# kemingy/rabitq

Hardware: AMD Instinct MI355X
Metric: queries/sec at recall@10>=0.95, 100Mx128; HBM GB/s on popcount scan (higher is better)
Workload: dtype exact integer dot (fp6 MFMA, v_dot8_u32_u4) + f32

## Files before the change

rabitq_amd/csrc/host_state.h:

```cpp
#pragma once
static thread_local std::string g_err;
static rq_status fail(rq_status s, const std::string &msg) {
    g_err = msg;
    return s;
}
#define HIPC(expr)                                                                                   \
    do {                                                                                             \
        hipError_t _e = (expr);                                                                      \
        if (_e != hipSuccess)                                                                        \
            return fail(_e == hipErrorOutOfMemory ? RQ_ERR_OOM : RQ_ERR_HIP,                         \
                        std::string(#expr) + ": " + hipGetErrorString(_e));                          \
    } while (0)
#define RQC(expr)                        \
    do {                                 \
        rq_status _s = (expr);           \
        if (_s != RQ_OK) return _s;      \
    } while (0)

static rq_status ensure_device() {
    int count = 0;
    hipError_t e = hipGetDeviceCount(&count);
    if (e != hipSuccess || count == 0)
        return fail(RQ_ERR_NO_DEVICE, "no HIP device visible (librabitq_hip has no CPU fallback)");
    return RQ_OK;
// ... 373 lines not shown
    if (cnt[b] == topk) {
        m = dist[(uint64_t)b * topk];
        for (uint32_t e = 1; e < topk; ++e) m = dist[(uint64_t)b * topk + e] > m ? dist[(uint64_t)b * topk + e] : m;
    }
    thr[b] = m;
}
__global__ void pack_topk_keys_at_kernel(const float *__restrict__ dist, const uint32_t *__restrict__ id, const uint32_t *__restrict__ cnt,
                                         uint32_t nq, uint32_t topk, uint32_t id_offset, uint32_t width, uint32_t col0,
                                         unsigned long long *__restrict__ keys) {
    const uint64_t i = (uint64_t)blockIdx.x * blockDim.x + threadIdx.x;
    if (i >= (uint64_t)nq * topk) return;
    const uint32_t b = (uint32_t)(i / topk), e = (uint32_t)(i - (uint64_t)b * topk);
    keys[(uint64_t)b * width + col0 + e] =
        e < cnt[b] ? (((unsigned long long)ord32_biased(dist[i]) << 32) | (uint32_t)(id[i] + id_offset)) : ~0ull;
}
__global__ void unpack_topk_keys_kernel(const unsigned long long *__restrict__ keys, uint32_t nq, uint32_t topk,
                                        float *__restrict__ dist, uint32_t *__restrict__ id, uint32_t *__restrict__ cnt) {
    const uint32_t b = blockIdx.x * blockDim.x + threadIdx.x;
    if (b >= nq) return;
    uint32_t c = 0;
    for (uint32_t e = 0; e < topk; ++e) {
        const unsigned long long key = keys[(uint64_t)b * topk + e];
        if (key == ~0ull) break;
        dist[(uint64_t)b * topk + e] = ord32_unbias((uint32_t)(key >> 32));
        id[(uint64_t)b * topk + e] = (uint32_t)key;
        ++c;
    }
    cnt[b] = c;
}

static std::atomic<int> g_coarse_impl{0};
static std::atomic<int> g_scan_dbg{0};
static bool select_is_wave(uint32_t k, uint32_t nprobe, uint32_t nq) { return nprobe <= 64 && k <= 4096 && nq >= 8; }
static void launch_coarse(const float *cent_t, const float *y, float *dist, uint32_t k, uint32_t dim, uint32_t nq,
                          uint32_t kstride, hipStream_t st) {
    const int impl = g_coarse_impl.load();
    const bool sreg = (impl == 2 || (impl == 0 && nq >= 2048)) && nq > 0;
    if (g_scan_dbg.load() & 16384)
        fprintf(stderr, "[rabitq_hip] plan: coarse=exact kernel=%s nq=%u k=%u\n", sreg ? "sreg" : (nq >= 64 && dim <= 2048 ? "lds8" : "lds4"), nq, k);
    if (sreg)
        coarse_dist_sreg_kernel<8><<<dim3(ceil_div(nq, 8), ceil_div(k, 256)), 256, 0, st>>>(cent_t, y, dist, k, dim, nq, kstride);
    else if (nq >= 64 && dim <= 2048)
        coarse_dist_kernel<8><<<dim3(ceil_div(nq, 8), ceil_div(k, 256)), 256, 8 * dim * sizeof(float), st>>>(cent_t, y, dist, k, dim, nq,
                                                                                                    kstride);
    else
        coarse_dist_kernel<4><<<dim3(ceil_div(nq, 4), ceil_div(k, 256)), 256, 4 * dim * sizeof(float), st>>>(cent_t, y, dist, k, dim, nq,
                                                                                                    kstride);
}

template <typename F>
static void with_row_kpl(uint32_t k, F f) {
    if (k <= 1024) f(std::integral_constant<int, 16>{});
    else if (k <= 4096) f(std::integral_constant<int, 64>{});
    else f(std::integral_constant<int, 128>{});
}
static void launch_select(const float *dist, uint32_t k, uint32_t nprobe, uint32_t *out_cluster, float *out_dist,
                          uint32_t id_offset, uint32_t out_stride, uint32_t nq, hipStream_t st) {
    if (select_is_wave(k, nprobe, nq)) {
        with_row_kpl(k, [&](auto kpl) {
            select_probe_wave_kernel<decltype(kpl)::value><<<ceil_div(nq, 4), 256, 0, st>>>(dist, k, nprobe, out_cluster, out_dist, id_offset, out_stride, nq);
        });
        return;
    }
    select_probe_kernel<<<nq, 256, (size_t)nprobe * 8, st>>>(dist, k, nprobe, out_cluster, out_dist, id_offset, out_stride);
}

static std::atomic<int> g_pair_split{1};
static std::atomic<int> g_coarse_tiled_from{4096};
static bool coarse_prefilter_has(uint32_t W) { return W == 1 || W == 2 || W == 3 || W == 4 || W == 6 || W == 8 || W == 12; }
static bool coarse_prefilter_applies(const rq_index *idx, uint32_t nq, uint32_t nprobe) {
    const int impl = g_coarse_impl.load();
    return (impl == 3 || impl == 4 || (impl == 0 && nq >= 2048)) && coarse_prefilter_has(idx->W) && std::isfinite(idx->cent_norm_max) &&
           idx->cent_bf.p != nullptr && nprobe <= 64 && nq >= 8 && idx->k >= 64 && nprobe >= 1 && idx->k <= 65536;
}
template <int W, int NT>
static size_t coarse_candidates_lds_bytes(uint32_t ntile) { return assign_lds_bytes<W, NT>() + (size_t)4 * NT * 32 * ntile * 4; }
#define RQ_LDS_PER_BLOCK (160u * 1024u)
static bool coarse_fused_applies(const rq_index *idx, uint32_t nprobe, bool have_redo) {
    const uint32_t k = idx->k, ntile = ceil_div(k, 32u);
    if (g_coarse_impl.load() != 0 || (g_scan_dbg.load() & 65536) || !have_redo || k < 4096 || k > 8192 || idx->W > 4 || ntile < nprobe) return false;
    const size_t images = 2 * (32 * ((size_t)idx->dim * 2 + 16) + 128);
    return images + (size_t)4 * 32 * ntile * 4 <= RQ_LDS_PER_BLOCK;
}
static void launch_coarse_prefiltered(const rq_index *idx, const float *y, float *dist, uint32_t nq, uint32_t nprobe, uint32_t *out_cluster,
                                      float *out_dist, uint32_t out_stride, unsigned long long *fallback_rows, uint32_t *redo, hipStream_t st,
                                      uint16_t *y_bf) {
    const uint32_t k = idx->k, dim = idx->dim;
    if (coarse_fused_applies(idx, nprobe, redo != nullptr)) {
        const uint32_t ntile = ceil_div(k, 32u);
        if (g_scan_dbg.load() & 16384) fprintf(stderr, "[rabitq_hip] plan: coarse=prefilter_fused nq=%u k=%u nprobe=%u\n", nq, k, nprobe);
#define RQ_CCK(WW, NT)                                                                                                                   \
    coarse_candidates_kernel<WW, NT><<<ceil_div(nq, 128 * NT), 256, coarse_candidates_lds_bytes<WW, NT>(ntile), st>>>(                   \
        y, idx->cent_bf.p, idx->cent_sqnorm.p, idx->cent_norm_max, nq, k, nprobe, dist, redo)
        if (idx->W == 1 && coarse_candidates_lds_bytes<1, 2>(ntile) <= RQ_LDS_PER_BLOCK) RQ_CCK(1, 2);
        else if (idx->W == 2 && coarse_candidates_lds_bytes<2, 2>(ntile) <= RQ_LDS_PER_BLOCK) RQ_CCK(2, 2);
        else if (idx->W == 1) RQ_CCK(1, 1);
        else if (idx->W == 2) RQ_CCK(2, 1);
        else if (idx->W == 3) RQ_CCK(3, 1);
        else RQ_CCK(4, 1);
#undef RQ_CCK
        refine_candidates_kernel<<<ceil_div(nq, 4), 256, 0, st>>>(dist, y, idx->centroids.p, k, dim, nprobe, out_cluster, out_dist, out_stride, nq, redo,
                                                                  fallback_rows);
        select_probe_kernel<<<nq, 256, (size_t)nprobe * 8, st>>>(dist, k, nprobe, out_cluster, out_dist, 0u, out_stride, redo);
        return;
    }
    if (idx->W > 8) to_bf16_kernel<<<ceil_div((uint64_t)nq * dim / 8, 256), 256, 0, st>>>(y, (uint64_t)nq * dim, y_bf);
#define RQ_CAP(WW, NT)                                                                                                      \
    coarse_approx_kernel<WW, NT><<<ceil_div(nq, 128 * NT), 256, assign_lds_bytes<WW, NT>(), st>>>(y, idx->cent_bf.p, idx->cent_sqnorm.p, nq, \
                                                                                                  k, dist, y_bf)
    switch (idx->W) {
        case 1: RQ_CAP(1, 2); break;
        case 2: RQ_CAP(2, 2); break;
        case 3: RQ_CAP(3, 1); break;
        case 4: RQ_CAP(4, 1); break;
        case 6: RQ_CAP(6, 1); break;
        case 8: RQ_CAP(8, 1); break;
        default: RQ_CAP(12, 1); break;
    }
#undef RQ_CAP
    const dim3 g(ceil_div(nq, 4)), b(256);
    const uint32_t ntile = ceil_div(k, 32u);
    const int impl = g_coarse_impl.load();
    const bool tiled = redo != nullptr && ntile >= nprobe &&
                       (k > 8192 || impl == 4 || (impl != 3 && k >= (uint32_t)g_coarse_tiled_from.load() && idx->W <= 8));
    if (g_scan_dbg.load() & 16384)
        fprintf(stderr, "[rabitq_hip] plan: coarse=%s nq=%u k=%u nprobe=%u\n", tiled ? "prefilter_tiled" : "prefilter_regs", nq, k, nprobe);
    if (tiled) {
#define RQ_TILED(TPL)                                                                                                             \
    select_refine_tiled_kernel<TPL><<<g, b, 4 * 64 * (TPL) * 4, st>>>(dist, y, idx->centroids.p, idx->cent_norm_max, k, dim, nprobe, out_cluster, \
                                                                    out_dist, out_stride, nq, redo, fallback_rows)
        if (ntile <= 128) RQ_TILED(2);
        else if (ntile <= 256) RQ_TILED(4);
        else if (ntile <= 512) RQ_TILED(8);
        else if (ntile <= 1024) RQ_TILED(16);
        else RQ_TILED(32);
#undef RQ_TILED
        select_probe_kernel<<<nq, 256, (size_t)nprobe * 8, st>>>(dist, k, nprobe, out_cluster, out_dist, 0u, out_stride, redo);
    } else {
        with_row_kpl(k, [&](auto kpl) {
            select_refine_wave_kernel<decltype(kpl)::value><<<g, b, 0, st>>>(dist, y, idx->centroids.p, idx->cent_norm_max, k, dim, nprobe, out_cluster, out_dist,
                                                                             out_stride, nq, fallback_rows);
        });
    }
}

#define RQ_MAX_BLOCKS_256 ((1u << 23) - 1)

static void launch_rotate(const float *x, const float *P, float *out, uint64_t n, uint32_t dim, bool mfma,
                          hipStream_t st) {
    const uint64_t rows_per_launch = mfma ? (1ull << 40) : (uint64_t)RQ_MAX_BLOCKS_256 * 4;
    for (uint64_t r0 = 0; r0 < n; r0 += rows_per_launch) {
        const uint64_t m = std::min(rows_per_launch, n - r0);
        const float *xs = x + r0 * dim;
        float *os = out + r0 * dim;
        if (mfma) {
            const uint32_t ncol = dim / ROT_BN;
            const uint64_t nrow_tiles = ceil_div(m, ROT_BM);
            const uint32_t groups = (uint32_t)std::min<uint64_t>(nrow_tiles, std::max<uint32_t>(1, 512 / ncol));
            rotate_mfma_kernel<<<dim3(groups * ncol), dim3(256), 0, st>>>(xs, P, os, m, dim, groups);
        } else {
            rotate_valu_kernel<<<dim3(ceil_div(m, 4), dim / 64), dim3(64, 4), 0, st>>>(xs, P, os, m, dim);
        }
    }
}

static const uint4 *get_tile_table(const rq_index *cidx, uint32_t tile, uint32_t *count) {
    rq_index *idx = const_cast<rq_index *>(cidx);
    std::lock_guard<std::mutex> lk(idx->tt_mu);
    auto it = idx->tile_tables.find(tile);
    if (it == idx->tile_tables.end()) {
        std::vector<uint4> h;
        h.reserve(idx->n / tile + idx->k + 1);
        for (uint32_t c = 0; c < idx->k; ++c) {
            const uint32_t b = idx->h_offsets[c], len = idx->h_offsets[c + 1] - b;
            for (uint32_t f = 0; f < len; f += tile) h.push_back(make_uint4(c, f, b, len));
        }
        std::unique_ptr<DevBuf<uint4>> buf(new DevBuf<uint4>());
        if (buf->alloc(h.size()) != RQ_OK) return nullptr;
        if (!h.empty() && hipMemcpy(buf->p, h.data(), h.size() * sizeof(uint4), hipMemcpyHostToDevice) != hipSuccess) return nullptr;
        buf->count = h.size();
        it = idx->tile_tables.emplace(tile, std::move(buf)).first;
    }
    *count = (uint32_t)it->second->count;
// ... 121 lines not shown
            default: break;
        }
    });
}
static void launch_scan_mfma(const ScanPtrs &p, const ScanArgs &args, uint32_t W, hipStream_t st, bool additive = false) {
    if (p.filtered) {
        if (p.arena) launch_scan_mfma_a<true, true>(p, args, W, st);
        else launch_scan_mfma_a<false, true>(p, args, W, st);
    } else if (p.arena) launch_scan_mfma_a<true>(p, args, W, st);
    else if (additive) launch_scan_mfma_add(p, args, W, st);
    else launch_scan_mfma_a<false>(p, args, W, st);
}

static bool scan_is_fused(uint32_t W) {
    switch (W) {
        case 1: case 2: case 3: case 4: case 6: case 8: case 12: case 16: return true;
        default: return false;
    }
}
static uint32_t scan_tile(uint32_t W) {
    switch (W) {
        case 1: case 2: case 3: case 4: case 6: case 8: return 512;
        default: return 256;
    }
}

template <int W, int NT>
static hipError_t set_scan_mfma_attr() {
    hipError_t e = hipFuncSetAttribute(reinterpret_cast<const void *>(scan_mfma_kernel<W, NT, false>),
                                       hipFuncAttributeMaxDynamicSharedMemorySize, (int)scan_mfma_ring_bytes(W));
    if (e != hipSuccess) return e;
    if constexpr (W <= 2) {
        e = hipFuncSetAttribute(reinterpret_cast<const void *>(scan_mfma_kernel<W, (W == 2 ? RQ_ADD_NT2 : NT), false, true>),
                                hipFuncAttributeMaxDynamicSharedMemorySize, (int)scan_mfma_ring_bytes(W));
        if (e != hipSuccess) return e;
    }
    e = hipFuncSetAttribute(reinterpret_cast<const void *>(scan_mfma_kernel<W, NT, true>),
                            hipFuncAttributeMaxDynamicSharedMemorySize, (int)scan_mfma_ring_bytes(W));
    if (e != hipSuccess) return e;
    e = hipFuncSetAttribute(reinterpret_cast<const void *>(scan_mfma_kernel<W, NT, false, false, true>),
                            hipFuncAttributeMaxDynamicSharedMemorySize, (int)scan_mfma_ring_bytes(W));
    if (e != hipSuccess) return e;
    return hipFuncSetAttribute(reinterpret_cast<const void *>(scan_mfma_kernel<W, NT, true, false, true>),
                               hipFuncAttributeMaxDynamicSharedMemorySize, (int)scan_mfma_ring_bytes(W));
}
void launch_sb_query_filtered(uint32_t W, int mode, uint32_t nq, size_t dyn, hipStream_t st, const SbArgs &sa);
hipError_t sb_query_filtered_set_attributes(int bytes);
static rq_status ensure_kernel_attributes() {
    static std::once_flag once;
    static hipError_t err = hipSuccess;
    static const char *what = "";
    std::call_once(once, [] {
        auto set = [&](const void *fn, int bytes, const char *name) {
            if (err != hipSuccess) return;
            err = hipFuncSetAttribute(fn, hipFuncAttributeMaxDynamicSharedMemorySize, bytes);
            if (err != hipSuccess) what = name;
        };
        set(reinterpret_cast<const void *>(select_probe_kernel), 140 * 1024, "select_probe_kernel");
        set(reinterpret_cast<const void *>(coarse_dist_kernel<4>), 140 * 1024, "coarse_dist_kernel<4>");
        set(reinterpret_cast<const void *>(coarse_dist_kernel<8>), 140 * 1024, "coarse_dist_kernel<8>");
        set(reinterpret_cast<const void *>(assign_generic_kernel<8>), 140 * 1024, "assign_generic_kernel<8>");
        set(reinterpret_cast<const void *>(merge_smallest_u64_kernel), 16384 * 8, "merge_smallest_u64_kernel");
        set(reinterpret_cast<const void *>(group_rank_kernel), 32768 * 4, "group_rank_kernel");
        set(reinterpret_cast<const void *>(sb_front_kernel), 140 * 1024, "sb_front_kernel");
        set(reinterpret_cast<const void *>(accurate_ring8_kernel<RQ_RING_V, 4>), 156 * 1024, "accurate_ring8_kernel<4>");
        set(reinterpret_cast<const void *>(accurate_ring8_kernel<RQ_RING_V, 8>), 156 * 1024, "accurate_ring8_kernel<8>");
        set(reinterpret_cast<const void *>(accurate_ring8_kernel<RQ_RING_V, 12>), 156 * 1024, "accurate_ring8_kernel<12>");
        set(reinterpret_cast<const void *>(accurate_ring8_kernel<RQ_RING_V, 16>), 156 * 1024, "accurate_ring8_kernel<16>");
        set(reinterpret_cast<const void *>(sort_runs_mid_kernel), RQ_SORT_MID_LDS_WORDS * 8, "sort_runs_mid_kernel");
        set(reinterpret_cast<const void *>(range_sort_block_kernel<1024, RQ_RANGE_TILE>), RQ_RANGE_TILE * 8, "range_sort_block_kernel");
        set(reinterpret_cast<const void *>(range_sort_tile_kernel), RQ_RANGE_TILE * 8, "range_sort_tile_kernel");
        set(reinterpret_cast<const void *>(assign_approx_kernel<6, 1>), (int)assign_lds_bytes<6, 1>(), "assign_approx_kernel<6,1>");
        set(reinterpret_cast<const void *>(assign_approx_kernel<8, 1>), (int)assign_lds_bytes<8, 1>(), "assign_approx_kernel<8,1>");
        set(reinterpret_cast<const void *>(assign_approx_kernel<12, 1>), (int)assign_lds_bytes<12, 1>(), "assign_approx_kernel<12,1>");
        set(reinterpret_cast<const void *>(coarse_approx_kernel<6, 1>), (int)assign_lds_bytes<6, 1>(), "coarse_approx_kernel<6,1>");
        set(reinterpret_cast<const void *>(coarse_approx_kernel<8, 1>), (int)assign_lds_bytes<8, 1>(), "coarse_approx_kernel<8,1>");
        set(reinterpret_cast<const void *>(coarse_approx_kernel<12, 1>), (int)assign_lds_bytes<12, 1>(), "coarse_approx_kernel<12,1>");
        set(reinterpret_cast<const void *>(coarse_candidates_kernel<1, 2>), (int)RQ_LDS_PER_BLOCK, "coarse_candidates_kernel<1,2>");
        set(reinterpret_cast<const void *>(coarse_candidates_kernel<2, 2>), (int)RQ_LDS_PER_BLOCK, "coarse_candidates_kernel<2,2>");
        set(reinterpret_cast<const void *>(coarse_candidates_kernel<1, 1>), (int)RQ_LDS_PER_BLOCK, "coarse_candidates_kernel<1,1>");
        set(reinterpret_cast<const void *>(coarse_candidates_kernel<2, 1>), (int)RQ_LDS_PER_BLOCK, "coarse_candidates_kernel<2,1>");
        set(reinterpret_cast<const void *>(coarse_candidates_kernel<3, 1>), (int)RQ_LDS_PER_BLOCK, "coarse_candidates_kernel<3,1>");
        set(reinterpret_cast<const void *>(coarse_candidates_kernel<4, 1>), (int)RQ_LDS_PER_BLOCK, "coarse_candidates_kernel<4,1>");
        set(reinterpret_cast<const void *>(sb_finish_kernel<true>), 104 * 1024, "sb_finish_kernel");
        set(reinterpret_cast<const void *>(sb_finish_kernel<false>), 104 * 1024, "sb_finish_kernel");
#define RQ_SBQ_ATTR(WW)                                                                                  \
    set(reinterpret_cast<const void *>(sb_query_kernel<WW, 0, false>), 120 * 1024, "sb_query_kernel");   \
    set(reinterpret_cast<const void *>(sb_query_kernel<WW, 1, false>), 120 * 1024, "sb_query_kernel");   \
    set(reinterpret_cast<const void *>(sb_query_kernel<WW, 2, false>), 120 * 1024, "sb_query_kernel")
        RQ_SBQ_ATTR(1);
        RQ_SBQ_ATTR(2);
        RQ_SBQ_ATTR(4);
        RQ_SBQ_ATTR(8);
        RQ_SBQ_ATTR(12);
        RQ_SBQ_ATTR(16);
#undef RQ_SBQ_ATTR
        if (err == hipSuccess && (err = sb_query_filtered_set_attributes(120 * 1024)) != hipSuccess) what = "sb_query_kernel (filtered)";
        auto chk = [&](hipError_t e, const char *name) {
            if (err == hipSuccess && e != hipSuccess) err = e, what = name;
        };
        chk(set_scan_mfma_attr<1, 4>(), "scan_mfma_kernel<1,4>");
        chk(set_scan_mfma_attr<2, RQ_NT_W2>(), "scan_mfma_kernel<2,NT>");
        chk(set_scan_mfma_attr<3, 4>(), "scan_mfma_kernel<3,4>");
        chk(set_scan_mfma_attr<4, 2>(), "scan_mfma_kernel<4,2>");
        chk(set_scan_mfma_attr<6, 2>(), "scan_mfma_kernel<6,2>");
        chk(set_scan_mfma_attr<8, 2>(), "scan_mfma_kernel<8,2>");
        chk(set_scan_mfma_attr<12, RQ_NT_W12>(), "scan_mfma_kernel<12,NT>");
        chk(set_scan_mfma_attr<16, 2>(), "scan_mfma_kernel<16,2>");
    });
    if (err != hipSuccess)
        return fail(RQ_ERR_HIP, std::string("hipFuncSetAttribute(") + what + "): " + hipGetErrorString(err));
    return RQ_OK;
}
```

rabitq_amd/csrc/kernels_coarse.h:

```cpp
#pragma once
#ifndef RQ_COLLECT_UNROLL
#define RQ_COLLECT_UNROLL 8
#endif
#include "common.h"

#pragma clang fp contract(off)

template <int QT>
__global__ __launch_bounds__(256) void coarse_dist_sreg_kernel(const float *__restrict__ cent_t,
                                                               const float *__restrict__ y, float *__restrict__ dist,
                                                               uint32_t k, uint32_t dim, uint32_t nq, uint32_t kstride) {
    const uint32_t q0 = blockIdx.x * QT;
    const uint32_t j = blockIdx.y * 256 + threadIdx.x;
    const bool live = j < k;
    const float *cp = cent_t + (live ? j : 0);
    f32x2 acc[QT][4];
#pragma unroll
    for (int v = 0; v < QT; ++v)
#pragma unroll
        for (int l = 0; l < 4; ++l) acc[v][l] = f32x2{0.0f, 0.0f};
    static_assert(QT % 4 == 0, "queries are fetched four at a time");
    for (uint32_t c = 0; c < dim; c += 16) {
        float ce[16];
#pragma unroll
// ... 614 lines not shown
            for (int i = 0; i < (int)(RQ_COARSE_CAND / 64); ++i) kk[i] = lane + 64 * i < base ? (uint32_t)(wn[lane + 64 * i] >> 32) : 0xFFFFFFFFu;
            const uint32_t h2 = bisect_loose(kmin, hi, nprobe, [&](uint32_t t) { return count_le(kk, t); });
            T2 = coarse_margin_key(yr, dim, cmax, ord32_unbias(h2));
            ok = T2 != 0xFFFFFFFFu && collect(T2);
        }
    }
    if (!ok || base < nprobe) {
        coarse_exact_row(centroids, yr, dim, k, d);
        if (lane == 0) {
            redo_flag[b] = 1u;
            if (fallback_rows) atomicAdd(fallback_rows, 1ull);
        }
        return;
    }
    if (lane == 0) redo_flag[b] = 0u;
    __builtin_amdgcn_fence(__ATOMIC_SEQ_CST, "wavefront");
    coarse_refine_tail(wn, base, centroids, yr, dim, nprobe, b, out_cluster, out_dist, out_stride);
}

template <int W, int NT>
__global__ __launch_bounds__(256, (W <= 4 ? 2 : 1)) void coarse_approx_kernel(const float *__restrict__ y ,
                                                              const uint16_t *__restrict__ cent_bf ,
                                                              const float *__restrict__ cnorm, uint32_t nq, uint32_t k,
                                                              float *__restrict__ dist ,
                                                              const uint16_t *__restrict__ y_bf ) {
    constexpr int DIM = 64 * W, NM = DIM / 16;
    constexpr uint32_t ROWB = CentTile<W>::ROWB, TILEB = CentTile<W>::TILEB;
    extern __shared__ __attribute__((aligned(16))) unsigned char asg_lds[];
    const uint32_t t = threadIdx.x, lane = t & 63, wave = t >> 6, col = lane & 31, kh = lane >> 5;
    const uint32_t v0 = (blockIdx.x * 4 + wave) * (32 * NT);
    asg_bf16x8 afrag[NT][NM];
#pragma unroll
    for (int tl = 0; tl < NT; ++tl) {
        const uint32_t v = v0 + 32 * tl + col;
        const uint64_t vr = v < nq ? v : (nq - 1);
        if constexpr (NM > 32) {
            const uint16_t *xb = y_bf + vr * DIM + 8 * kh;
#pragma unroll
            for (int m = 0; m < NM; ++m) afrag[tl][m] = __builtin_bit_cast(asg_bf16x8, *reinterpret_cast<const uint4 *>(xb + 16 * m));
        } else {
        const float *xp = y + vr * DIM + 8 * kh;
#pragma unroll
        for (int m = 0; m < NM; ++m) {
            const float4 a = *reinterpret_cast<const float4 *>(xp + 16 * m), b = *reinterpret_cast<const float4 *>(xp + 16 * m + 4);
            const uint4 pk = make_uint4(asg_bf16_pair(a.x, a.y), asg_bf16_pair(a.z, a.w), asg_bf16_pair(b.x, b.y), asg_bf16_pair(b.z, b.w));
            afrag[tl][m] = __builtin_bit_cast(asg_bf16x8, pk);
        }
        }
    }
    const uint32_t ntile = (k + 31) / 32;
    CentTile<W> next;
    next.stage(cent_bf, cnorm, k, 0, 0.0f);
    next.land(asg_lds, 0);
    for (uint32_t tile = 0; tile < ntile; ++tile) {
        __syncthreads();
        if (tile + 1 < ntile) next.stage(cent_bf, cnorm, k, tile + 1, 0.0f);
        const unsigned char *img = CentTile<W>::image(asg_lds, tile & 1u);
        const float cn = reinterpret_cast<const float *>(img + TILEB)[col];
        asg_f32x16 acc[NT];
#pragma unroll
        for (int tl = 0; tl < NT; ++tl) acc[tl] = asg_f32x16{0, 0, 0, 0, 0, 0, 0, 0, 0, 0, 0, 0, 0, 0, 0, 0};
#pragma unroll
        for (int m = 0; m < NM; ++m) {
            const asg_bf16x8 cf = *reinterpret_cast<const asg_bf16x8 *>(img + col * ROWB + (16 * m + 8 * kh) * 2);
#pragma unroll
            for (int tl = 0; tl < NT; ++tl) acc[tl] = __builtin_amdgcn_mfma_f32_32x32x16_bf16(afrag[tl][m], cf, acc[tl], 0, 0, 0);
        }
        const uint32_t j = 32 * tile + col;
        if (j < k) {
#pragma unroll
            for (int tl = 0; tl < NT; ++tl)
#pragma unroll
                for (int r = 0; r < 16; ++r) {
                    const uint32_t v = v0 + 32 * tl + (uint32_t)((r & 3) + 8 * (r >> 2)) + 4 * kh;
                    if (v < nq) dist[(uint64_t)v * k + j] = fmaf(-2.0f, acc[tl][r], cn);
                }
        }
        if (tile + 1 < ntile) next.land(asg_lds, (tile + 1) & 1u);
    }
}

#define RQ_COARSE_PAD_NORM 3.0e38f
#define RQ_FUSED_WINDOW 4u
template <int W, int NT>
__global__ __launch_bounds__(256) void coarse_candidates_kernel(const float *__restrict__ y ,
                                                                const uint16_t *__restrict__ cent_bf ,
                                                                const float *__restrict__ cnorm, float cmax, uint32_t nq, uint32_t k,
                                                                uint32_t nprobe, float *__restrict__ dist ,
                                                                uint32_t *__restrict__ cand_cnt ) {
    constexpr int DIM = 64 * W, NM = DIM / 16;
    constexpr uint32_t ROWB = CentTile<W>::ROWB, TILEB = CentTile<W>::TILEB;
    extern __shared__ __attribute__((aligned(16))) unsigned char asg_lds[];
    const uint32_t t = threadIdx.x, lane = t & 63, wave = t >> 6, col = lane & 31, kh = lane >> 5;
    const uint32_t ntile = (k + 31) / 32;
    uint32_t *tkeys = reinterpret_cast<uint32_t *>(asg_lds + 2 * (TILEB + 128)) + wave * (NT * 32) * ntile;
    const uint32_t v0 = (blockIdx.x * 4 + wave) * (32 * NT);
    asg_bf16x8 bfrag[NT][NM];
    float yn[NT];
#pragma unroll
    for (int tl = 0; tl < NT; ++tl) {
        const uint32_t v = v0 + 32 * tl + col;
        const float *xp = y + (uint64_t)(v < nq ? v : (nq - 1)) * DIM + 8 * kh;
        float s0 = 0.0f, s1 = 0.0f;
#pragma unroll
        for (int m = 0; m < NM; ++m) {
            const float4 a = *reinterpret_cast<const float4 *>(xp + 16 * m), b = *reinterpret_cast<const float4 *>(xp + 16 * m + 4);
            s0 = fmaf(a.x, a.x, s0), s1 = fmaf(a.y, a.y, s1), s0 = fmaf(a.z, a.z, s0), s1 = fmaf(a.w, a.w, s1);
            s0 = fmaf(b.x, b.x, s0), s1 = fmaf(b.y, b.y, s1), s0 = fmaf(b.z, b.z, s0), s1 = fmaf(b.w, b.w, s1);
            const uint4 pk = make_uint4(asg_bf16_pair(a.x, a.y), asg_bf16_pair(a.z, a.w), asg_bf16_pair(b.x, b.y), asg_bf16_pair(b.z, b.w));
            bfrag[tl][m] = __builtin_bit_cast(asg_bf16x8, pk);
        }
        const float s = s0 + s1;
        yn[tl] = s + __shfl_xor(s, 32, 64);
    }
    float thr[NT];
    bool fin[NT];
    uint32_t kmin[NT], kmax[NT], cnt[NT];
#pragma unroll
    for (int tl = 0; tl < NT; ++tl) thr[tl] = 0.0f, fin[tl] = false, kmin[tl] = 0xFFFFFFFFu, kmax[tl] = 0u, cnt[tl] = 0u;
    for (int pass = 0; pass < 2; ++pass) {
        CentTile<W> next;
        __syncthreads();
        next.stage(cent_bf, cnorm, k, 0, RQ_COARSE_PAD_NORM);
        next.land(asg_lds, 0);
        for (uint32_t tile = 0; tile < ntile; ++tile) {
            __syncthreads();
            if (tile + 1 < ntile) next.stage(cent_bf, cnorm, k, tile + 1, RQ_COARSE_PAD_NORM);
            const unsigned char *img = CentTile<W>::image(asg_lds, tile & 1u);
            const float *cnp = reinterpret_cast<const float *>(img + TILEB);
            asg_f32x16 acc[NT];
#pragma unroll
            for (int tl = 0; tl < NT; ++tl) acc[tl] = asg_f32x16{0, 0, 0, 0, 0, 0, 0, 0, 0, 0, 0, 0, 0, 0, 0, 0};
#pragma unroll
            for (int m = 0; m < NM; ++m) {
                const asg_bf16x8 af = *reinterpret_cast<const asg_bf16x8 *>(img + col * ROWB + (16 * m + 8 * kh) * 2);
#pragma unroll
                for (int tl = 0; tl < NT; ++tl) acc[tl] = __builtin_amdgcn_mfma_f32_32x32x16_bf16(af, bfrag[tl][m], acc[tl], 0, 0, 0);
            }
            float cnr[16];
#pragma unroll
            for (int g = 0; g < 4; ++g) {
                const float4 c4 = *reinterpret_cast<const float4 *>(cnp + 8 * g + 4 * kh);
                cnr[4 * g] = c4.x, cnr[4 * g + 1] = c4.y, cnr[4 * g + 2] = c4.z, cnr[4 * g + 3] = c4.w;
            }
            const bool ragged = 32 * tile + 32 > k;
#pragma unroll
            for (int tl = 0; tl < NT; ++tl) {
                if (pass == 0) {
                    float mn = __builtin_inff();
#pragma unroll
                    for (int r = 0; r < 16; ++r) mn = fminf(mn, fmaf(-2.0f, acc[tl][r], cnr[r]));
                    mn = fminf(mn, __shfl_xor(mn, 32, 64));
                    const uint32_t key = ord32_biased(mn);
                    kmin[tl] = key < kmin[tl] ? key : kmin[tl];
                    kmax[tl] = key > kmax[tl] ? key : kmax[tl];
                    if (kh == 0) tkeys[(tl * ntile + tile) * 32 + col] = key;
                } else {
                    uint32_t mine = 0;
#pragma unroll
                    for (int r = 0; r < 16; ++r) mine |= fmaf(-2.0f, acc[tl][r], cnr[r]) <= thr[tl] ? (1u << r) : 0u;
                    if (ragged) {
#pragma unroll
                        for (int r = 0; r < 16; ++r)
                            if (32 * tile + (uint32_t)((r & 3) + 8 * (r >> 2)) + 4 * kh >= k) mine &= ~(1u << r);
                    }
                    if (!fin[tl]) mine = 0;
                    const uint32_t other = (uint32_t)__shfl_xor((int)mine, 32, 64);
                    const uint32_t c_mine = (uint32_t)__popc(mine), c_other = (uint32_t)__popc(other);
                    uint32_t at = cnt[tl] + (kh ? c_other : 0u);
                    cnt[tl] += c_mine + c_other;
                    uint16_t *cand = reinterpret_cast<uint16_t *>(tkeys + tl * ntile * 32) + col * RQ_COARSE_CAND;
                    while (mine) {
                        const uint32_t r = (uint32_t)__builtin_ctz(mine);
                        mine &= mine - 1u;
                        if (at < RQ_COARSE_CAND) cand[at] = (uint16_t)(32 * tile + (r & 3u) + 8u * (r >> 2) + 4u * kh);
                        ++at;
                    }
                }
            }
            if (tile + 1 < ntile) next.land(asg_lds, (tile + 1) & 1u);
        }
        if (pass == 0) {
            __builtin_amdgcn_fence(__ATOMIC_SEQ_CST, "wavefront");
#pragma unroll
            for (int tl = 0; tl < NT; ++tl) {
                const uint32_t *tk = tkeys + tl * ntile * 32 + col;
                uint32_t lo = kmin[tl], hi = kmax[tl];
                bool open = lo < hi;
                while (__ballot(open)) {
                    const uint32_t mid = lo + ((hi - lo) >> 1);
                    uint32_t c = 0;
#pragma unroll 16
                    for (uint32_t i = kh; i < ntile; i += 2) c += tk[i * 32] <= mid ? 1u : 0u;
                    c += (uint32_t)__shfl_xor((int)c, 32, 64);
                    if (open) {
                        if (c >= nprobe) {
                            hi = mid;
                            if (c <= nprobe + RQ_FUSED_WINDOW) open = false;
                        } else {
                            lo = mid + 1;
                        }
                        open = open && lo < hi;
                    }
                }
                const float tau = ord32_unbias(hi);
                const float t2 = prefilter_bound(tau, cmax, yn[tl], DIM);
                fin[tl] = fabsf(t2) < 3.0e38f && fabsf(tau) < 3.0e38f;
                thr[tl] = t2;
            }
        }
    }
    __builtin_amdgcn_fence(__ATOMIC_SEQ_CST, "wavefront");
#pragma unroll
    for (int tl = 0; tl < NT; ++tl) {
        const uint32_t v = v0 + 32 * tl + col;
        const uint32_t cval = fin[tl] ? cnt[tl] : 0xFFFFFFFFu;
        if (kh == 0 && v < nq) cand_cnt[v] = cval;
        const uint16_t *cand = reinterpret_cast<const uint16_t *>(tkeys + tl * ntile * 32);
        for (uint32_t qi = 0; qi < 32; ++qi) {
            const uint32_t c = (uint32_t)__shfl((int)cval, (int)qi, 64), vq = v0 + 32 * tl + qi;
            if (vq >= nq || c > RQ_COARSE_CAND) continue;
            uint32_t *slots = reinterpret_cast<uint32_t *>(dist + (uint64_t)vq * k);
            for (uint32_t s = lane; s < c; s += 64) slots[s] = cand[qi * RQ_COARSE_CAND + s];
        }
    }
}

__global__ __launch_bounds__(256) void refine_candidates_kernel(float *__restrict__ dist, const float *__restrict__ y,
                                                                const float *__restrict__ centroids, uint32_t k, uint32_t dim, uint32_t nprobe,
                                                                uint32_t *__restrict__ out_cluster, float *__restrict__ out_dist,
                                                                uint32_t out_stride, uint32_t nq, uint32_t *__restrict__ cnt_flag,
                                                                unsigned long long *__restrict__ fallback_rows ) {
    __shared__ unsigned long long win[4][RQ_COARSE_CAND];
    const uint32_t wave = threadIdx.x >> 6, lane = threadIdx.x & 63, b = blockIdx.x * 4 + wave;
    if (b >= nq) return;
    unsigned long long *wn = win[wave];
    float *d = dist + (uint64_t)b * k;
    const float *yr = y + (uint64_t)b * dim;
    const uint32_t c2 = __builtin_amdgcn_readfirstlane(cnt_flag[b]);
    if (c2 > RQ_COARSE_CAND || c2 < nprobe) {
        coarse_exact_row(centroids, yr, dim, k, d);
        if (lane == 0) {
            cnt_flag[b] = 1u;
            if (fallback_rows) atomicAdd(fallback_rows, 1ull);
        }
        return;
    }
    const uint32_t *slots = reinterpret_cast<const uint32_t *>(d);
    for (uint32_t i = lane; i < c2; i += 64) wn[i] = slots[i];
    if (lane == 0) cnt_flag[b] = 0u;
    __builtin_amdgcn_fence(__ATOMIC_SEQ_CST, "wavefront");
    coarse_refine_tail(wn, c2, centroids, yr, dim, nprobe, b, out_cluster, out_dist, out_stride);
}
```

rabitq_amd/csrc/rabitq_hip.hip:

```cpp
#include "../../include/rabitq_hip.h"

#include <hip/hip_runtime.h>

#include <algorithm>
#include <charconv>
#include <chrono>
#include <atomic>
#include <cmath>
#include <cstdio>
#include <cstdlib>
#include <cstring>
#include <memory>
#include <mutex>
#include <random>
#include <string>
#include <thread>
#include <vector>
#include <sys/stat.h>
#include <dlfcn.h>
#include <queue>
#include <map>

#include "common.h"
#include "kernels_build.h"
// ... 912 lines not shown
        if (value < 0) return fail(RQ_ERR_INVALID, "max_scan_blocks must be >= 0");
        g_max_scan_blocks = value == 0 ? RQ_MAX_BLOCKS_256 : std::min<uint32_t>((uint32_t)value, RQ_MAX_BLOCKS_256);
        return RQ_OK;
    }
    if (std::string(name) == "pair_split") {
        if (value < 0 || value > 1) return fail(RQ_ERR_INVALID, "pair_split must be 0 or 1");
        g_pair_split = value;
        return RQ_OK;
    }
    if (std::string(name) == "coarse_tiled_from") {
        if (value < 0) return fail(RQ_ERR_INVALID, "coarse_tiled_from must be >= 0");
        g_coarse_tiled_from = value;
        return RQ_OK;
    }
    if (std::string(name) == "coarse_impl") {
        if (value < 0 || value > 4) return fail(RQ_ERR_INVALID, "coarse_impl must be 0, 1, 2, 3 or 4");
        g_coarse_impl = value;
        return RQ_OK;
    }
    if (std::string(name) == "survivor_segments") {
#ifdef RQ_DEV_ABLATIONS
        if (value < 0 || value > 3) return fail(RQ_ERR_INVALID, "survivor_segments must be 0, 1, 2 or 3");
#else
        if (value == 3) return fail(RQ_ERR_INVALID, "survivor_segments = 3 (allocation-failure injection) exists in the developer build only (make dev)");
        if (value < 0 || value > 2) return fail(RQ_ERR_INVALID, "survivor_segments must be 0, 1 or 2");
#endif
        g_seg_opt = value;
        return RQ_OK;
    }
    if (std::string(name) == "assign_impl") {
        if (value < 0 || value > 1) return fail(RQ_ERR_INVALID, "assign_impl must be 0 or 1");
        g_assign_impl = value;
        return RQ_OK;
    }
    if (std::string(name) == "small_batch_span") {
        if (value < 1) return fail(RQ_ERR_INVALID, "small_batch_span must be >= 1");
        g_sb_span = value;
        return RQ_OK;
    }
    if (std::string(name) == "small_batch") {
        if (value < 0 || value > 1) return fail(RQ_ERR_INVALID, "small_batch must be 0 or 1");
        g_small_batch = value;
        return RQ_OK;
    }
    if (std::string(name) == "small_batch_filtered") {
        if (value < 0 || value > 2) return fail(RQ_ERR_INVALID, "small_batch_filtered must be 0, 1 or 2");
        g_sb_filtered = value;
        return RQ_OK;
    }
    if (std::string(name) == "dense_dir") {
        if (value < 0 || value > 1) return fail(RQ_ERR_INVALID, "dense_dir must be 0 or 1");
        g_dense_dir = value;
        return RQ_OK;
    }
    if (std::string(name) == "shared_thresholds") {
        if (value < 0 || value > 2) return fail(RQ_ERR_INVALID, "shared_thresholds must be 0, 1 or 2");
        g_shared_thr = value;
        return RQ_OK;
    }
    if (std::string(name) == "group_rank") {
        if (value < 0 || value > 2) return fail(RQ_ERR_INVALID, "group_rank must be 0, 1 or 2");
        g_group_rank = value;
        return RQ_OK;
    }
    if (std::string(name) == "prep_placement") {
        if (value < 0 || value > 1) return fail(RQ_ERR_INVALID, "prep_placement must be 0 or 1");
        g_prep_placement = value;
        return RQ_OK;
    }
    if (std::string(name) == "rerank_shadow") {
        if (value < 0 || value > 2) return fail(RQ_ERR_INVALID, "rerank_shadow must be 0 (never), 1 (fp16 rows when they fit) or 2 (8-bit rows when they fit)");
        g_rerank_shadow = value;
        return RQ_OK;
    }
    if (std::string(name) == "scan_gate") {
        if (value < 0 || value > 2) return fail(RQ_ERR_INVALID, "scan_gate must be 0, 1 or 2");
        g_scan_gate = value;
        return RQ_OK;
    }
    if (std::string(name) == "scan_debug") {
#ifdef RQ_DEV_ABLATIONS
        const int allowed = 0x7FFFFFFF;
#else
        const int allowed = 128 | 512 | 2048 | 4096 | 16384 | 32768 | 65536;
#endif
        if (value < 0 || (value & ~allowed)) return fail(RQ_ERR_INVALID, "scan_debug: this bit exists in the developer build only (librabitq_hip_dev.so)");
        g_scan_dbg = value;
        return RQ_OK;
    }
    return fail(RQ_ERR_INVALID, std::string("unknown option ") + name);
}

rq_status rq_set_profiling(int level) {
    if (level < 0 || level > 2) return fail(RQ_ERR_INVALID, "profiling level must be 0, 1 or 2");
    g_profiling = level;
    return RQ_OK;
}
rq_status rq_last_profile(rq_profile_t *out) {
    if (!out) return fail(RQ_ERR_INVALID, "null argument");
    return copy_out_sized(out, g_profile);
}

rq_status rq_rotate(const float *x, uint64_t n, uint32_t dim, const float *orthogonal, int use_mfma, float *out) {
    RQC(ensure_device());
    if (!x || !orthogonal || !out) return fail(RQ_ERR_INVALID, "null argument");
    if (dim == 0 || dim % 64) return fail(RQ_ERR_DIM_MISMATCH, "dim must be a multiple of 64");
    DevBuf<float> dx, dp, dout;
    RQC(dx.upload(x, n * dim));
    RQC(dp.upload(orthogonal, (size_t)dim * dim));
    RQC(dout.alloc(n * dim));
    launch_rotate(dx.p, dp.p, dout.p, n, dim, use_mfma != 0, nullptr);
    HIPC(hipDeviceSynchronize());
    HIPC(hipGetLastError());
    HIPC(hipMemcpy(out, dout.p, n * dim * 4, hipMemcpyDeviceToHost));
    return RQ_OK;
}

rq_status rq_rotate_device(const rq_index *idx, const float *d_x, uint64_t n, float *d_out, float *out_ms) {
    RQC(ensure_device());
    if (!idx || !d_x || !d_out) return fail(RQ_ERR_INVALID, "null argument");
    hipEvent_t e0, e1;
    HIPC(hipEventCreate(&e0));
    HIPC(hipEventCreate(&e1));
    HIPC(hipEventRecord(e0, nullptr));
    launch_rotate(d_x, idx->P.p, d_out, n, idx->dim, true, nullptr);
    HIPC(hipEventRecord(e1, nullptr));
    HIPC(hipEventSynchronize(e1));
    HIPC(hipGetLastError());
    float ms = 0;
    HIPC(hipEventElapsedTime(&ms, e0, e1));
    if (out_ms) *out_ms = ms;
    (void)hipEventDestroy(e0);
    (void)hipEventDestroy(e1);
    return RQ_OK;
}

rq_status rq_quantize_pack(const float *x_rot, uint64_t n, uint32_t dim, const float *centroids_rot, uint32_t k,
                           uint32_t *out_label, float *out_dist, uint64_t *out_codes, rq_factor_t *out_factors) {
    RQC(ensure_device());
    RQC(ensure_kernel_attributes());
    if (!x_rot || !centroids_rot || !out_label || !out_dist || !out_codes || !out_factors)
        return fail(RQ_ERR_INVALID, "null argument");
    if (dim == 0 || dim % 64 || k == 0) return fail(RQ_ERR_DIM_MISMATCH, "dim must be a multiple of 64, k > 0");
    rq_index tmp;
    tmp.dim = dim, tmp.k = k, tmp.W = dim / 64;
    DevBuf<float> dx, dd;
    DevBuf<uint32_t> dl;
    DevBuf<uint64_t> dc;
    DevBuf<float4> df;
    RQC(dx.upload(x_rot, n * dim));
    RQC(tmp.centroids.upload(centroids_rot, (size_t)k * dim));
    RQC(tmp.cent_t.alloc((size_t)k * dim));
    RQC(dd.alloc(n));
    RQC(dl.alloc(n));
    RQC(dc.alloc(n * tmp.W));
    RQC(df.alloc(n));
    transpose_kernel<<<dim3(ceil_div(dim, 32), ceil_div(k, 32)), dim3(32, 8)>>>(tmp.centroids.p, tmp.cent_t.p, k, dim);
    AssignAux ax;
    HIPC(hipDeviceSynchronize());
    if (assign_has_mfma(tmp.W) && g_assign_impl.load() != 1) RQC(assign_aux_init(&tmp, ax, std::min<uint64_t>(std::max<uint64_t>(n, 1), 1ull << 20)));
    for (uint64_t i0 = 0; i0 < n; i0 += (1ull << 20)) {
        const uint64_t m = std::min<uint64_t>(1ull << 20, n - i0);
        RQC(launch_assign_prefiltered(dx.p + i0 * dim, &tmp, ax, m, dl.p + i0, dd.p + i0));
        quantize_kernel<<<ceil_div(m, 32), 256>>>(dx.p + i0 * dim, tmp.centroids.p, dl.p + i0, m, dim,
                                                  dc.p + i0 * tmp.W, df.p + i0);
    }
    HIPC(hipDeviceSynchronize());
// ... 113 lines not shown
```

Baseline: 4.052 million.

## Add wide 512-thread coarse candidate kernel with triple-buffered centroid ring

Adds a new fused coarse-candidate kernel for W=1/2 that uses 8 waves per block, each wave handling 32 queries. All waves share a three-slot LDS ring of centroid tiles filled by async global-to-LDS loads. The kernel makes two sweeps, one for tile keys and one for threshold-filtered candidates, and overlaps the MFMA products with prefetch of tiles two steps ahead. This is meant to amortise centroid loads across more queries and to hide load latency. The cost is more barriers and more LDS per block, which may reduce occupancy. A debug bit can disable the new path.

After: 4.046 million. No clear change (-0.2%).

```diff
diff --git a/rabitq_amd/csrc/host_state.h b/rabitq_amd/csrc/host_state.h
--- a/rabitq_amd/csrc/host_state.h
+++ b/rabitq_amd/csrc/host_state.h
@@ -479,23 +479,35 @@
     const size_t images = 2 * (32 * ((size_t)idx->dim * 2 + 16) + 128);
     return images + (size_t)4 * 32 * ntile * 4 <= RQ_LDS_PER_BLOCK;
 }
+static size_t coarse_wide_lds_bytes(uint32_t dim, uint32_t ntile) { return 3 * ((size_t)64 * dim + 128) + (size_t)8 * 32 * ntile * 4; }
+static bool coarse_wide_applies(const rq_index *idx) {
+    return !(g_scan_dbg.load() & 131072) && (idx->W == 1 || idx->W == 2) && coarse_wide_lds_bytes(idx->dim, ceil_div(idx->k, 32u)) <= RQ_LDS_PER_BLOCK;
+}
 static void launch_coarse_prefiltered(const rq_index *idx, const float *y, float *dist, uint32_t nq, uint32_t nprobe, uint32_t *out_cluster,
                                       float *out_dist, uint32_t out_stride, unsigned long long *fallback_rows, uint32_t *redo, hipStream_t st,
                                       uint16_t *y_bf) {
     const uint32_t k = idx->k, dim = idx->dim;
     if (coarse_fused_applies(idx, nprobe, redo != nullptr)) {
         const uint32_t ntile = ceil_div(k, 32u);
-        if (g_scan_dbg.load() & 16384) fprintf(stderr, "[rabitq_hip] plan: coarse=prefilter_fused nq=%u k=%u nprobe=%u\n", nq, k, nprobe);
+        const bool wide = coarse_wide_applies(idx);
+        if (g_scan_dbg.load() & 16384)
+            fprintf(stderr, "[rabitq_hip] plan: coarse=prefilter_fused nq=%u k=%u nprobe=%u geom=%s\n", nq, k, nprobe, wide ? "wide" : "narrow");
+#define RQ_CCW(WW)                                                                                                                       \
+    coarse_candidates_wide_kernel<WW><<<ceil_div(nq, 256), 512, coarse_wide_lds_bytes(dim, ntile), st>>>(                                \
+        y, idx->cent_bf.p, idx->cent_sqnorm.p, idx->cent_norm_max, nq, k, nprobe, dist, redo)
 #define RQ_CCK(WW, NT)                                                                                                                   \
     coarse_candidates_kernel<WW, NT><<<ceil_div(nq, 128 * NT), 256, coarse_candidates_lds_bytes<WW, NT>(ntile), st>>>(                   \
         y, idx->cent_bf.p, idx->cent_sqnorm.p, idx->cent_norm_max, nq, k, nprobe, dist, redo)
-        if (idx->W == 1 && coarse_candidates_lds_bytes<1, 2>(ntile) <= RQ_LDS_PER_BLOCK) RQ_CCK(1, 2);
+        if (wide && idx->W == 1) RQ_CCW(1);
+        else if (wide) RQ_CCW(2);
+        else if (idx->W == 1 && coarse_candidates_lds_bytes<1, 2>(ntile) <= RQ_LDS_PER_BLOCK) RQ_CCK(1, 2);
         else if (idx->W == 2 && coarse_candidates_lds_bytes<2, 2>(ntile) <= RQ_LDS_PER_BLOCK) RQ_CCK(2, 2);
         else if (idx->W == 1) RQ_CCK(1, 1);
         else if (idx->W == 2) RQ_CCK(2, 1);
         else if (idx->W == 3) RQ_CCK(3, 1);
         else RQ_CCK(4, 1);
 #undef RQ_CCK
+#undef RQ_CCW
         refine_candidates_kernel<<<ceil_div(nq, 4), 256, 0, st>>>(dist, y, idx->centroids.p, k, dim, nprobe, out_cluster, out_dist, out_stride, nq, redo,
                                                                   fallback_rows);
         select_probe_kernel<<<nq, 256, (size_t)nprobe * 8, st>>>(dist, k, nprobe, out_cluster, out_dist, 0u, out_stride, redo);
@@ -783,6 +795,8 @@
         set(reinterpret_cast<const void *>(coarse_candidates_kernel<2, 1>), (int)RQ_LDS_PER_BLOCK, "coarse_candidates_kernel<2,1>");
         set(reinterpret_cast<const void *>(coarse_candidates_kernel<3, 1>), (int)RQ_LDS_PER_BLOCK, "coarse_candidates_kernel<3,1>");
         set(reinterpret_cast<const void *>(coarse_candidates_kernel<4, 1>), (int)RQ_LDS_PER_BLOCK, "coarse_candidates_kernel<4,1>");
+        set(reinterpret_cast<const void *>(coarse_candidates_wide_kernel<1>), (int)RQ_LDS_PER_BLOCK, "coarse_candidates_wide_kernel<1>");
+        set(reinterpret_cast<const void *>(coarse_candidates_wide_kernel<2>), (int)RQ_LDS_PER_BLOCK, "coarse_candidates_wide_kernel<2>");
         set(reinterpret_cast<const void *>(sb_finish_kernel<true>), 104 * 1024, "sb_finish_kernel");
         set(reinterpret_cast<const void *>(sb_finish_kernel<false>), 104 * 1024, "sb_finish_kernel");
 #define RQ_SBQ_ATTR(WW)                                                                                  \
diff --git a/rabitq_amd/csrc/kernels_coarse.h b/rabitq_amd/csrc/kernels_coarse.h
--- a/rabitq_amd/csrc/kernels_coarse.h
+++ b/rabitq_amd/csrc/kernels_coarse.h
@@ -720,6 +720,93 @@
 
 #define RQ_COARSE_PAD_NORM 3.0e38f
 #define RQ_FUSED_WINDOW 4u
+template <int NM>
+__device__ __forceinline__ float coarse_cand_query(const float *__restrict__ y, uint32_t v, uint32_t nq, uint32_t kh, asg_bf16x8 (&bfrag)[NM]) {
+    const float *xp = y + (uint64_t)(v < nq ? v : (nq - 1)) * (16 * NM) + 8 * kh;
+    float s0 = 0.0f, s1 = 0.0f;
+#pragma unroll
+    for (int m = 0; m < NM; ++m) {
+        const float4 a = *reinterpret_cast<const float4 *>(xp + 16 * m), b = *reinterpret_cast<const float4 *>(xp + 16 * m + 4);
+        s0 = fmaf(a.x, a.x, s0), s1 = fmaf(a.y, a.y, s1), s0 = fmaf(a.z, a.z, s0), s1 = fmaf(a.w, a.w, s1);
+        s0 = fmaf(b.x, b.x, s0), s1 = fmaf(b.y, b.y, s1), s0 = fmaf(b.z, b.z, s0), s1 = fmaf(b.w, b.w, s1);
+        const uint4 pk = make_uint4(asg_bf16_pair(a.x, a.y), asg_bf16_pair(a.z, a.w), asg_bf16_pair(b.x, b.y), asg_bf16_pair(b.z, b.w));
+        bfrag[m] = __builtin_bit_cast(asg_bf16x8, pk);
+    }
+    const float s = s0 + s1;
+    return s + __shfl_xor(s, 32, 64);
+}
+__device__ __forceinline__ void coarse_cand_norms(const float *cnp, uint32_t kh, float (&cnr)[16]) {
+#pragma unroll
+    for (int g = 0; g < 4; ++g) {
+        const float4 c4 = *reinterpret_cast<const float4 *>(cnp + 8 * g + 4 * kh);
+        cnr[4 * g] = c4.x, cnr[4 * g + 1] = c4.y, cnr[4 * g + 2] = c4.z, cnr[4 * g + 3] = c4.w;
+    }
+}
+__device__ __forceinline__ uint32_t coarse_cand_tile_key(const asg_f32x16 &acc, const float (&cnr)[16]) {
+    float mn = __builtin_inff();
+#pragma unroll
+    for (int r = 0; r < 16; ++r) mn = fminf(mn, fmaf(-2.0f, acc[r], cnr[r]));
+    mn = fminf(mn, __shfl_xor(mn, 32, 64));
+    return ord32_biased(mn);
+}
+__device__ __forceinline__ void coarse_cand_append(const asg_f32x16 &acc, const float (&cnr)[16], float thr, bool fin, uint32_t tile, uint32_t k,
+                                                   uint32_t kh, uint32_t &cnt, uint16_t *cand) {
+    uint32_t mine = 0;
+#pragma unroll
+    for (int r = 0; r < 16; ++r) mine |= fmaf(-2.0f, acc[r], cnr[r]) <= thr ? (1u << r) : 0u;
+    if (32 * tile + 32 > k) {
+#pragma unroll
+        for (int r = 0; r < 16; ++r)
+            if (32 * tile + (uint32_t)((r & 3) + 8 * (r >> 2)) + 4 * kh >= k) mine &= ~(1u << r);
+    }
+    if (!fin) mine = 0;
+    const uint32_t other = (uint32_t)__shfl_xor((int)mine, 32, 64);
+    const uint32_t c_mine = (uint32_t)__popc(mine), c_other = (uint32_t)__popc(other);
+    uint32_t at = cnt + (kh ? c_other : 0u);
+    cnt += c_mine + c_other;
+    while (mine) {
+        const uint32_t r = (uint32_t)__builtin_ctz(mine);
+        mine &= mine - 1u;
+        if (at < RQ_COARSE_CAND) cand[at] = (uint16_t)(32 * tile + (r & 3u) + 8u * (r >> 2) + 4u * kh);
+        ++at;
+    }
+}
+__device__ __forceinline__ void coarse_cand_threshold(const uint32_t *tk, uint32_t ntile, uint32_t kh, uint32_t kmin, uint32_t kmax, uint32_t nprobe,
+                                                      float cmax, float yn, uint32_t dim, float &thr, bool &fin) {
+    uint32_t lo = kmin, hi = kmax;
+    bool open = lo < hi;
+    while (__ballot(open)) {
+        const uint32_t mid = lo + ((hi - lo) >> 1);
+        uint32_t c = 0;
+#pragma unroll 16
+        for (uint32_t i = kh; i < ntile; i += 2) c += tk[i * 32] <= mid ? 1u : 0u;
+        c += (uint32_t)__shfl_xor((int)c, 32, 64);
+        if (open) {
+            if (c >= nprobe) {
+                hi = mid;
+                if (c <= nprobe + RQ_FUSED_WINDOW) open = false;
+            } else {
+                lo = mid + 1;
+            }
+            open = open && lo < hi;
+        }
+    }
+    const float tau = ord32_unbias(hi);
+    thr = prefilter_bound(tau, cmax, yn, dim);
+    fin = fabsf(thr) < 3.0e38f && fabsf(tau) < 3.0e38f;
+}
+__device__ __forceinline__ void coarse_cand_flush(const uint16_t *cand, uint32_t v0, uint32_t cval, uint32_t nq, uint32_t k, float *__restrict__ dist,
+                                                  uint32_t *__restrict__ cand_cnt) {
+    const uint32_t lane = threadIdx.x & 63;
+    if (lane < 32 && v0 + lane < nq) cand_cnt[v0 + lane] = cval;
+    for (uint32_t qi = 0; qi < 32; ++qi) {
+        const uint32_t c = (uint32_t)__shfl((int)cval, (int)qi, 64), vq = v0 + qi;
+        if (vq >= nq || c > RQ_COARSE_CAND) continue;
+        uint32_t *slots = reinterpret_cast<uint32_t *>(dist + (uint64_t)vq * k);
+        for (uint32_t s = lane; s < c; s += 64) slots[s] = cand[qi * RQ_COARSE_CAND + s];
+    }
+}
+
 template <int W, int NT>
 __global__ __launch_bounds__(256) void coarse_candidates_kernel(const float *__restrict__ y ,
                                                                 const uint16_t *__restrict__ cent_bf ,
@@ -864,6 +951,119 @@
     }
 }
 
+template <int W>
+struct CentRing {
+    static constexpr int DIM = 64 * W;
+    static constexpr uint32_t PPR = DIM / 8, ROWSB = 32 * DIM * 2, IMGB = ROWSB + 128;
+    static constexpr uint32_t LANES = 32 * PPR / 8;
+    static_assert(W == 1 || W == 2, "one copy of at most 64 lanes per wave and tile");
+    static __device__ __forceinline__ uint32_t piece(uint32_t row, uint32_t g) { return W == 2 ? g ^ (row & 15u) : g ^ ((row >> 1) & 7u); }
+    static __device__ __forceinline__ uint32_t uniform(uint32_t v) { return __builtin_amdgcn_readfirstlane(v); }
+    static __device__ __forceinline__ void issue(const uint16_t *__restrict__ cent_bf, const float *__restrict__ cnorm, uint32_t k, uint32_t tile,
+                                                 uint32_t img, uint32_t wave, uint32_t lane) {
+        if (LANES == 64 || lane < LANES) {
+            const uint32_t p = wave * LANES + lane, row = p / PPR, j = 32 * tile + row;
+            glds16(cent_bf + (uint64_t)(j < k ? j : k - 1) * DIM + 8 * piece(row, p % PPR), uniform(img + 16 * LANES * wave));
+        }
+        if (lane == 0) {
+            const uint32_t j0 = 32 * tile + 4 * wave;
+            glds16(cnorm + (j0 + 4 <= k ? j0 : 0u), uniform(img + ROWSB + 16 * wave));
+        }
+    }
+};
+__device__ __forceinline__ void coarse_ring_barrier() { asm volatile("s_waitcnt lgkmcnt(0)\n\ts_barrier" ::: "memory"); }
+template <int W>
+__global__ __launch_bounds__(512) void coarse_candidates_wide_kernel(const float *__restrict__ y ,
+                                                                     const uint16_t *__restrict__ cent_bf ,
+                                                                     const float *__restrict__ cnorm, float cmax, uint32_t nq, uint32_t k,
+                                                                     uint32_t nprobe, float *__restrict__ dist ,
+                                                                     uint32_t *__restrict__ cand_cnt ) {
+    using Ring = CentRing<W>;
+    constexpr int DIM = 64 * W, NM = DIM / 16;
+    extern __shared__ __attribute__((aligned(16))) unsigned char asg_lds[];
+    const uint32_t t = threadIdx.x, lane = t & 63, wave = __builtin_amdgcn_readfirstlane(t >> 6), col = lane & 31, kh = lane >> 5;
+    const uint32_t ntile = (k + 31) / 32;
+    uint32_t *tkeys = reinterpret_cast<uint32_t *>(asg_lds + 3 * Ring::IMGB) + wave * 32 * ntile;
+    uint16_t *cand = reinterpret_cast<uint16_t *>(tkeys);
+    const uint32_t ring = lds_addr(asg_lds);
+    const uint32_t v0 = (blockIdx.x * 8 + wave) * 32;
+    asg_bf16x8 bfrag[NM];
+    const float yn = coarse_cand_query<NM>(y, v0 + col, nq, kh, bfrag);
+    float thr = 0.0f;
+    bool fin = false;
+    uint32_t kmin = 0xFFFFFFFFu, kmax = 0u, cnt = 0u;
+    uint32_t slot = 0;
+    auto enter = [&](uint32_t tile) -> const unsigned char * {
+        if (tile + 1 < ntile) asm volatile("s_waitcnt vmcnt(2)" ::: "memory");
+        else asm volatile("s_waitcnt vmcnt(0)" ::: "memory");
+        coarse_ring_barrier();
+        unsigned char *img = asg_lds + slot * Ring::IMGB;
+        if (32 * tile + 32 > k) {
+            if (t < 32) reinterpret_cast<float *>(img + Ring::ROWSB)[t] = 32 * tile + t < k ? cnorm[32 * tile + t] : RQ_COARSE_PAD_NORM;
+            coarse_ring_barrier();
+        }
+        slot = slot == 2 ? 0u : slot + 1u;
+        return img;
+    };
+    auto refill = [&](uint32_t tile) {
+        if (tile + 2 < ntile) Ring::issue(cent_bf, cnorm, k, tile + 2, ring + (slot == 2 ? 0u : slot + 1u) * Ring::IMGB, wave, lane);
+    };
+    auto product = [&](const unsigned char *img, asg_f32x16 &acc, float (&cnr)[16]) {
+        acc = asg_f32x16{0, 0, 0, 0, 0, 0, 0, 0, 0, 0, 0, 0, 0, 0, 0, 0};
+#pragma unroll
+        for (int m = 0; m < NM; ++m) {
+            const asg_bf16x8 af = *reinterpret_cast<const asg_bf16x8 *>(img + col * (DIM * 2) + 16 * Ring::piece(col, 2 * m + kh));
+            acc = __builtin_amdgcn_mfma_f32_32x32x16_bf16(af, bfrag[m], acc, 0, 0, 0);
+        }
+        coarse_cand_norms(reinterpret_cast<const float *>(img + Ring::ROWSB), kh, cnr);
+    };
+    auto sweep = [&](auto pass_c) {
+        constexpr int PASS = decltype(pass_c)::value;
+        auto finish = [&](uint32_t tile, const asg_f32x16 &acc, const float (&cnr)[16]) {
+            if constexpr (PASS == 0) {
+                const uint32_t key = coarse_cand_tile_key(acc, cnr);
+                kmin = key < kmin ? key : kmin;
+                kmax = key > kmax ? key : kmax;
+                if (kh == 0) tkeys[tile * 32 + col] = key;
+            } else {
+                coarse_cand_append(acc, cnr, thr, fin, tile, k, kh, cnt, cand + col * RQ_COARSE_CAND);
+            }
+        };
+        coarse_ring_barrier();
+        slot = 0;
+        Ring::issue(cent_bf, cnorm, k, 0, ring, wave, lane);
+        Ring::issue(cent_bf, cnorm, k, 1, ring + Ring::IMGB, wave, lane);
+        if constexpr (PASS == 1) {
+            __builtin_amdgcn_fence(__ATOMIC_SEQ_CST, "wavefront");
+            coarse_cand_threshold(tkeys + col, ntile, kh, kmin, kmax, nprobe, cmax, yn, DIM, thr, fin);
+        }
+        asg_f32x16 acc_a, acc_b;
+        float cn_a[16], cn_b[16];
+        product(enter(0), acc_a, cn_a);
+        refill(0);
+        uint32_t tile = 1;
+        for (; tile + 1 < ntile; tile += 2) {
+            product(enter(tile), acc_b, cn_b);
+            refill(tile);
+            finish(tile - 1, acc_a, cn_a);
+            product(enter(tile + 1), acc_a, cn_a);
+            refill(tile + 1);
+            finish(tile, acc_b, cn_b);
+        }
+        if (tile < ntile) {
+            product(enter(tile), acc_b, cn_b);
+            finish(tile - 1, acc_a, cn_a);
+            finish(tile, acc_b, cn_b);
+        } else {
+            finish(tile - 1, acc_a, cn_a);
+        }
+    };
+    sweep(std::integral_constant<int, 0>{});
+    sweep(std::integral_constant<int, 1>{});
+    __builtin_amdgcn_fence(__ATOMIC_SEQ_CST, "wavefront");
+    coarse_cand_flush(cand, v0, fin ? cnt : 0xFFFFFFFFu, nq, k, dist, cand_cnt);
+}
+
 __global__ __launch_bounds__(256) void refine_candidates_kernel(float *__restrict__ dist, const float *__restrict__ y,
                                                                 const float *__restrict__ centroids, uint32_t k, uint32_t dim, uint32_t nprobe,
                                                                 uint32_t *__restrict__ out_cluster, float *__restrict__ out_dist,
diff --git a/rabitq_amd/csrc/rabitq_hip.hip b/rabitq_amd/csrc/rabitq_hip.hip
--- a/rabitq_amd/csrc/rabitq_hip.hip
+++ b/rabitq_amd/csrc/rabitq_hip.hip
@@ -1018,7 +1018,7 @@
 #ifdef RQ_DEV_ABLATIONS
         const int allowed = 0x7FFFFFFF;
 #else
-        const int allowed = 128 | 512 | 2048 | 4096 | 16384 | 32768 | 65536;
+        const int allowed = 128 | 512 | 2048 | 4096 | 16384 | 32768 | 65536 | 131072;
 #endif
         if (value < 0 || (value & ~allowed)) return fail(RQ_ERR_INVALID, "scan_debug: this bit exists in the developer build only (librabitq_hip_dev.so)");
         g_scan_dbg = value;
```
